# HuiHuiLan/Clustering-Hidden-Markov-Models-with-Variational-Bayesian-Hierarchical-EM

Hardware: AMD Instinct MI355X
Metric: VBHEM E-steps/sec (whole node), N baseHMMs × K clusters × S states; ELBO match (higher is better)
Workload: dtype f64; 1 GPU; C4: N=100000 base HMMs, K=16 clusters, S=8 states, Sb=8, d=8, full cov, tau=10, Nv=100; N=100000, K=16, S=8, Sb=8, d=8, tau=10, parallelism=bases sharded over 1 GPU(s), 1 RCCL all-reduce/E-step

## Files before the change

clustering-hidden-markov-models-with-variational-bayesian-hierarchical-em_amd/csrc/vbhem_capi.hip:

```cpp
#include <hip/hip_runtime.h>

#include <algorithm>
#include <atomic>
#include <chrono>
#include <cmath>
#include <cstdio>
#include <cstring>
#include <cstdlib>
#include <random>
#include <string>
#include <utility>
#include <vector>

#include "vbhem_estep.h"
#include "vbhem_internal.h"
#include "vbhem_exact.h"
#include "vbhem_math.h"

static std::atomic<size_t> g_debug_extra_lds{0};

namespace {

thread_local std::string g_err;

struct TimingState {
  int level = 0;
  std::vector<std::pair<hipEvent_t, hipEvent_t>> fb, stats, em, gf, emd;
  std::vector<long long> fb_pairs;
  std::vector<hipEvent_t> pool;
  ~TimingState() {
    for (hipEvent_t e : pool) (void)hipEventDestroy(e);
  }
};
thread_local TimingState g_timing;

thread_local std::string g_last_kernel[2];
std::string split_name(const vbhem::SplitArgs &a) {
  return "vbhem::fb_split_kernel<" + std::to_string(a.S) + ", " + std::to_string(a.lpc) + ", " +
         std::to_string(a.mode) + ">";
}

struct SwitchRow {
  const char *name;
  long long unset;
  long long vbhem::Switches::*field;
};
constexpr SwitchRow kSwitchRows[] = {
#define X(name, unset, doc) {"VBHEM_" #name, unset, &vbhem::Switches::name},
    VBHEM_SWITCHES(X)
#undef X
};
// ... 304 lines not shown
                     : nullptr;
  w.scratch = cv.take<double>(exact_stride(c->S, b->SB, T) * kExactThreads);
  return cv.off + 256;
}

struct FusedWs {
  int group;
  int nslab;
  int slab_len;
  int *fpre, *flags;
  int *gate_cnt, *list, *list_tot;
  double *Atg;
  double *scratch, *nu1, *xi, *tnu, *Z, *slabs;
  double *E, *W, *bias, *shift;
  double *U;
};

size_t carve_fused(void *ws, const vbhem_base_t *b, const vbhem_cluster_t *c, int T, FusedWs &w,
                   int R = 1) {
  Carver cv(ws);
  const int K = c->K, S = c->S, SB = b->SB;
  const size_t per_base = (size_t)K * (S + (size_t)S * S + 2 * (size_t)S * SB) * sizeof(double);
  size_t g = std::max<size_t>(1, kGroupBudget / std::max<size_t>(1, per_base));
  g = std::min<size_t>(g, (size_t)std::max(1, b->N));
  const vbhem::Switches &sw = vbhem::switches();
  if (sw.GROUP_BASES >= 0)
    g = std::max<size_t>(1, std::min<size_t>(g, (size_t)sw.GROUP_BASES));
  w.group = (int)g;
  int maxslab = kMaxSlabs;
  if (sw.NSLAB >= 0) maxslab = (int)std::max(1ll, std::min(8192ll, sw.NSLAB));
// ... 4 lines not shown
  w.nu1 = cv.take<double>(g * K * S);
  w.xi = cv.take<double>(g * K * S * S);
  w.tnu = cv.take<double>(g * K * S * SB);
  w.Z = cv.take<double>(g * K);
  w.slabs = cv.take<double>((size_t)w.nslab * w.slab_len);
  w.E = cv.take<double>(g * K * S * SB);
  w.W = cv.take<double>(emission_w_doubles(b->d, b->covmode, K, S));
  w.bias = cv.take<double>((size_t)vbhem::emission_ksp(K * S));
  w.shift = cv.take<double>((size_t)b->d);
  w.U = need_u_ws(b) ? cv.take<double>(vbhem::u_doubles((long long)g * SB + 16, b->d, b->covmode))
                     : nullptr;
  w.gate_cnt = cv.take<int>((size_t)w.nslab * K);
  w.list = cv.take<int>(g * K);
  w.list_tot = cv.take<int>((size_t)K);
  w.Atg = cv.take<double>((size_t)K * S * S);
  w.scratch = cv.take<double>(exact_stride(S, SB, T) * kExactThreads);
  return cv.off + 256;
}

struct FbCtx {
  FbPlan plan;
  SplitPlan split;
  SplitPlan bwd;
  size_t bwd2_lds = 0;
  int bwd2_ppb = 0, bwd2_nwb = 0;
  bool bwd12 = false;
  bool bwd4 = false;
  bool list4 = false;
  bool list12 = false;
  bool k1_in_kernel = false;
// ... 81 lines not shown
  c.em.Atg = Atg; c.em.logA = logA;
  hipError_t e = vbhem::launch_emission_prep(c.em, st);
  if (e != hipSuccess) return hip_fail(e, "emission_prep_kernel");
  return VBHEM_OK;
}

unsigned list_grid(const vbhem::SplitArgs &a, size_t lds) {
  const int cus = vbhem::device_cus();
  const int per_cu = std::max(1, vbhem::split_resident_blocks(a, lds));
  return (unsigned)(cus * per_cu);
}

int run_fb_list(const FbCtx &c, int i_begin, int i_end, int i_buf0, double *nu1, double *xi,
                double *tnu, const double *Ebuf, long long e_ld, const int *list,
                const int *list_tot, int list_cap, int *flags, double *scratch, double *LL,
                hipStream_t st, bool fold = false, bool *inlined = nullptr) {
  if (i_end <= i_begin) return VBHEM_OK;
  if (!c.split.lds_l) return fail(VBHEM_ERR_UNSUPPORTED, "gate-list pass does not fit LDS");
  vbhem::SplitArgs ca = c.split.al;
  ca.mode = vbhem::kFbList;
  ca.E = Ebuf; ca.e_ld = e_ld;
  ca.i_begin = i_begin; ca.i_end = i_end; ca.i_buf0 = i_buf0;
  ca.LL = nullptr; ca.nu1 = nu1; ca.xi = xi; ca.tnu = tnu;
  ca.flag_count = flags; ca.flag_list = flags + vbhem::kFlagHead;
  ca.list = list; ca.list_tot = list_tot; ca.list_cap = list_cap;
  ca.xinline = 0;
  auto set_inline = [&](long long waves) {
    if (!fold || waves > kExactThreads || vbhem::switches().NO_LIST_INLINE) return;
    ca.xinline = 1;
    ca.xscr = scratch;
    ca.xstride = (long long)exact_stride(c.plan.a.S, c.plan.a.SB, c.plan.a.T);
    vbhem::FbArgs &x = ca.xf;
    x = c.plan.a;
    x.i_begin = i_begin; x.i_end = i_end; x.i_buf0 = i_buf0;
    x.LL = LL; x.nu1 = nu1; x.xi = xi; x.tnu = tnu;
    x.flag_count = flags; x.flag_list = flags + vbhem::kFlagHead;
  };
  hipEvent_t ev0 = timing_on(st) ? timing_event(st) : nullptr;
  hipError_t e;
  if (c.list4) {
    ca.Atg = c.bwd.a.Atg;
    const unsigned grid = (unsigned)(vbhem::device_cus() * std::max(1, vbhem::list4_resident_blocks()));
    set_inline(vbhem::list4_inline_waves(ca, grid));
    e = vbhem::launch_list4(ca, grid, st);
    if (e != hipSuccess) return hip_fail(e, "fb_list4_kernel");
    g_last_kernel[1] = "vbhem::fb_list4_kernel<" + std::to_string(ca.T) +
                       (vbhem::list4_fast(ca) ? ", true>" : ", false>");
  } else if (c.list12) {
    ca.Atg = c.bwd.a.Atg;
    const unsigned grid = (unsigned)(vbhem::device_cus() * std::max(1, vbhem::list12_resident_blocks()));
    e = vbhem::launch_list12(ca, grid, st);
    if (e != hipSuccess) return hip_fail(e, "fb_list12_kernel");
    g_last_kernel[1] = "vbhem::fb_list12_kernel<" + std::to_string(ca.T) +
                       (vbhem::list12_fast(ca) ? ", true>" : ", false>");
  } else {
    if (c.k1_in_kernel) set_k1_operands(c, i_begin, ca);
    const unsigned grid = list_grid(ca, c.split.lds_l);
    if (ca.S >= vbhem::kSplitInlineMinS && ca.S <= vbhem::kSplitInlineMaxS)
// ... 139 lines not shown
  }
  e = vbhem::launch_fb_exact(a, scratch, exact_stride(a.S, a.SB, a.T), kExactThreads, st);
  if (e != hipSuccess) return hip_fail(e, "fb_exact_kernel");
  return VBHEM_OK;
}

}

extern "C" {

const char *vbhem_last_error(void) { return g_err.c_str(); }

size_t vbhem_debug_extra_lds(size_t bytes) { return g_debug_extra_lds.exchange(bytes); }

const char *vbhem_last_kernel(int pass) {
  return (pass == 0 || pass == 1) ? g_last_kernel[pass].c_str() : "";
}

const char *vbhem_version(void) { return "vbhem-mi355x 0.1.0 (gfx950)"; }

size_t vbhem_stats_nu(int d, int covmode) {
  return covmode == VBHEM_COV_FULL ? (size_t)1 + d + (size_t)d * (d + 1) / 2 : (size_t)1 + 2 * d;
}

size_t vbhem_stats_len(int K, int S, int d, int covmode) {
  return (size_t)K + (size_t)K * S + (size_t)K * S * S + 2 + (size_t)K * S * vbhem_stats_nu(d, covmode);
}

size_t vbhem_prepare_base_bytes(const vbhem_base_t *base) {
  if (!base || base->N < 0 || base->SB < 1 || base->d < 1 || base->d > vbhem::kUHead ||
      (base->covmode != VBHEM_COV_DIAG && base->covmode != VBHEM_COV_FULL))
// ... 284 lines not shown
        sa.U = base->U; sa.uz = base->U; sa.u_col0 = 0;
        sa.Us = base->U + vbhem::u_doubles((long long)base->N * SB, base->d, base->covmode);
      } else if (ctx.u_ws) {
        sa.U = ctx.u_ws; sa.uz = ctx.em.shift; sa.u_col0 = (long long)g0 * SB / 16 * 16;
      }
    }
    const int nchunk = std::max(1, chunks(g1 - g0));
    hipEvent_t ev0 = timing_on(st) ? timing_event(st) : nullptr;
    e = vbhem::launch_resp(sa, nchunk, st);
    if (e != hipSuccess) return hip_fail(e, "resp_kernel");
    if (gated) {
      e = vbhem::launch_gate_list(sa, nchunk, st);
      if (e != hipSuccess) return hip_fail(e, "gate_list_kernel");
      if (ev0) g_timing.stats.emplace_back(ev0, timing_event(st));
      bool inl = false;
      rc = run_fb_list(ctx, g0, g1, g0, w.nu1, w.xi, w.tnu, w.E, e_ld, w.list, w.list_tot,
                       w.group, w.flags, w.scratch, LL_elbo_dev, st, fold, &inl);
      if (rc != VBHEM_OK) return rc;
      if (fold) sa.fold = inl ? 2 : 1;
      ev0 = timing_on(st) ? timing_event(st) : nullptr;
      int ss = nchunk;
      e = vbhem::launch_stats_list(sa, nchunk, sl_lds, st, &ss);
      if (e != hipSuccess) return hip_fail(e, "stats_list_kernel");
      if (g0 == 0) stats_slabs = ss;
    } else {
      e = vbhem::launch_stats(sa, nchunk, ngroups, slds, st);
      if (e != hipSuccess) return hip_fail(e, "stats_kernel");
    }
    if (ev0) g_timing.stats.emplace_back(ev0, timing_event(st));
  }
  e = vbhem::launch_stats_final(w.slabs, nslab_used, stats_slabs, w.slab_len, sa.KT, S, sa.SL,
                                stats_dev, st, w.fpre, done_word, done_val);
  if (e != hipSuccess) return hip_fail(e, "stats_final_kernel");
  guard.fpre = nullptr;
  return VBHEM_OK;
}

// ... 426 lines not shown
```

clustering-hidden-markov-models-with-variational-bayesian-hierarchical-em_amd/csrc/vbhem_fb_list4.hip:

```cpp
#include <hip/hip_runtime.h>

#include <algorithm>
#include <cmath>
#include <type_traits>

#include "vbhem_exact.h"
#include "vbhem_internal.h"
#include "vbhem_math.h"
#include "vbhem_mfma4.h"


namespace vbhem {

namespace {
using namespace m4;
constexpr int kL4Waves = 2;
constexpr int kL4NWB = 4;
constexpr int kL4T = 10;
}
constexpr int kL4XQ = 1024;
namespace {
}

template <int T, bool FAST>
__global__ __launch_bounds__(64 * kL4NWB) __attribute__((amdgpu_waves_per_eu(kL4Waves)))
void fb_list4_kernel(const SplitArgs p) {
  constexpr int S = 8;
  __shared__ __attribute__((aligned(16))) double etab[2048];
  __shared__ __attribute__((aligned(16))) double ltab[2 * 1024];
  __shared__ int pre[kList4MaxK + 1];
  __shared__ int tots[kList4MaxK];
  __shared__ int xq[kL4NWB * kL4XQ];
  const int tid = threadIdx.x;
  stage_tables(etab, ltab, tid, 64 * kL4NWB);
  const int K = p.K, SB = FAST ? 8 : p.SB;
  using off_t_ = typename std::conditional<FAST, unsigned, size_t>::type;
  auto ld = [](const double *base, off_t_ x) {
    if constexpr (FAST)
      return *reinterpret_cast<const double *>(reinterpret_cast<const char *>(base) + x * 8u);
    else
      return base[x];
  };
  if (tid == 0) {
    int s = 0;
    for (int jj = 0; jj < K; ++jj) {
      const int t = p.list_tot[jj];
      pre[jj] = s;
      tots[jj] = t;
      s += (t + 3) / 4;
    }
    pre[K] = s;
  }
  __syncthreads();
  const int nitem = __builtin_amdgcn_readfirstlane(pre[K]);
  const double vlim = kVMax / (double)T - 3.0;
  const int gw = (int)blockIdx.x * kL4NWB + (tid >> 6), nw = (int)gridDim.x * kL4NWB;

  struct ItemIn {
    double ab[2][2], e[2][2], pr[2], af[2][2];
  };
  auto load_in = [&](int i, int jj, int r_, int c_, ItemIn &in) {
#pragma unroll
    for (int j2 = 0; j2 < 2; ++j2)
#pragma unroll
      for (int j3 = 0; j3 < 2; ++j3) {
        const int be = 4 * j3 + c_, bp = 4 * j2 + r_;
        const int bec = be < SB ? be : SB - 1, bpc = bp < SB ? bp : SB - 1;
        in.ab[j2][j3] = ld(p.A, ((off_t_)i * SB + bec) * SB + bpc);
        in.af[j2][j3] = ld(p.A, ((off_t_)i * SB + bpc) * SB + bec);
      }
#pragma unroll
// ... 6 lines not shown
      }
#pragma unroll
    for (int j3 = 0; j3 < 2; ++j3) {
      const int be = 4 * j3 + c_;
      in.pr[j3] = ld(p.prior, (off_t_)i * SB + (be < SB ? be : SB - 1));
    }
  };
  auto base_of = [&](int it, int jj, int b_) -> int {
    const int n0 = (it - pre[jj]) * 4;
    const int tot = tots[jj];
    return p.list[(size_t)jj * p.list_cap + (n0 + b_ < tot ? n0 + b_ : n0)];
  };
  int js = 0, jsn = 0, nq = 0;
  ItemIn cur;
  int icur = 0;
  if (gw < nitem) {
    const int lane = tid & 63;
    while (pre[js + 1] <= gw) ++js;
    jsn = js;
    icur = base_of(gw, __builtin_amdgcn_readfirstlane(js), (lane >> 2) & 3);
    load_in(icur, __builtin_amdgcn_readfirstlane(js), lane >> 4, lane & 3, cur);
  }
  for (int it = gw; it < nitem; it += nw) {
    int tq = tid;
    asm volatile("" : "+v"(tq));
    const int lane = tq & 63;
    const int r = lane >> 4, b = (lane >> 2) & 3, c = lane & 3;
    const int qsrc0 = (4 * b + r) << 2, qsrc1 = (16 + 4 * b + r) << 2;
    const int taddr = (16 * c + 4 * b + r) << 2;
    const unsigned long long pmask = 0x000F000F000F000Full << (4 * b);
    const int j = __builtin_amdgcn_readfirstlane(js);
    const int itn = min(it + nw, nitem - 1);
    while (pre[jsn + 1] <= itn) ++jsn;
    const int jn = __builtin_amdgcn_readfirstlane(jsn);
    const int inext = base_of(itn, jn, b);
    double AT[2][2], Ap[2][2], amQ[2], lpP[2];
    bool cl_nf;
    {
      const double *At = p.Atg + (size_t)j * S * S;
      bool nf = false;
#pragma unroll
      for (int x = 0; x < 2; ++x)
#pragma unroll
        for (int y = 0; y < 2; ++y) {
          AT[x][y] = At[(4 * y + c) * S + 4 * x + r];
          Ap[x][y] = At[(4 * x + r) * S + 4 * y + c];
        }
// ... 125 lines not shown
        wpf[x] = 2147483648u - kBias;
      }
      exp_m_n<4>(ef, xf, sf, wpf, etab);
#pragma unroll
      for (int jj = 0; jj < 2; ++jj) {
        const int be = 4 * jj + c;
        const double pb = be < SB ? cur.pr[jj] : 0.0;
        nu[0][jj] = pb * ef[jj];
        nu[1][jj] = pb * ef[2 + jj];
      }
#pragma unroll
      for (int i2 = 0; i2 < 2; ++i2) {
        double a = nu[i2][0] + nu[i2][1];
        a += shfl_xor_d(a, 1);
        a += shfl_xor_d(a, 2);
        if (act && c == 0) p.nu1[lp * S + 4 * i2 + r] = a;
      }
    }

    double AbF[2][2];
#pragma unroll
    for (int j2 = 0; j2 < 2; ++j2)
#pragma unroll
      for (int jj = 0; jj < 2; ++jj) {
        const int bp = 4 * j2 + r, be = 4 * jj + c;
        AbF[j2][jj] = (be < SB && bp < SB) ? cur.af[j2][jj] : 0.0;
      }
    ItemIn nxt;
    double nuT[2][2], tnT[2][2], H[2][2];
    transpose8(nu, nuT, taddr);
#pragma unroll
    for (int x = 0; x < 2; ++x)
#pragma unroll
      for (int y = 0; y < 2; ++y) {
        tnT[x][y] = nuT[x][y];
        H[x][y] = 0.0;
      }
#pragma unroll
    for (int t = 1; t < T; ++t) {
      if (t == T / 2) load_in(inext, jn, r, c, nxt);
      double Gt[2][2];
      transpose8(lat[t], Gt, taddr);
      double fT[2][2], ZT[2][2];
#pragma unroll
      for (int jj = 0; jj < 2; ++jj)
#pragma unroll
        for (int i2 = 0; i2 < 2; ++i2) {
          fT[jj][i2] = mfma4(AbF[1][jj], nuT[1][i2], mfma4(AbF[0][jj], nuT[0][i2], 0.0));
          ZT[jj][i2] = mfma4(lat[t][1][jj], AT[1][i2], mfma4(lat[t][0][jj], AT[0][i2], 0.0));
        }
      double gT[2][2];
      {
        const double zf[4] = {ZT[0][0], ZT[0][1], ZT[1][0], ZT[1][1]};
        double rz[4];
        rcp_pos_n<4>(rz, zf);
// ... 6 lines not shown
        for (int i3 = 0; i3 < 2; ++i3) H[i2][i3] = mfma4(gT[1][i2], Gt[1][i3], mfma4(gT[0][i2], Gt[0][i3], H[i2][i3]));
      double g[2][2];
      transpose8(gT, g, taddr);
#pragma unroll
      for (int jj = 0; jj < 2; ++jj)
#pragma unroll
        for (int i3 = 0; i3 < 2; ++i3) {
          const double qm = mfma4(g[1][jj], Ap[1][i3], mfma4(g[0][jj], Ap[0][i3], 0.0));
          nuT[jj][i3] = Gt[jj][i3] * qm;
          tnT[jj][i3] += nuT[jj][i3];
        }
    }

    const bool pbad = (__ballot(bad) & pmask) != 0;
    const bool pnf = cl_nf || (__ballot(nfp) & pmask) != 0;
    if (act) {
#pragma unroll
      for (int jj = 0; jj < 2; ++jj)
#pragma unroll
        for (int i2 = 0; i2 < 2; ++i2) {
          const int be = 4 * jj + r;
          if (be < SB) p.tnu[(lp * S + 4 * i2 + c) * SB + be] = tnT[jj][i2];
        }
#pragma unroll
      for (int i2 = 0; i2 < 2; ++i2)
#pragma unroll
        for (int i3 = 0; i3 < 2; ++i3) p.xi[(lp * S + 4 * i2 + r) * S + 4 * i3 + c] = Ap[i2][i3] * H[i2][i3];
      if (pbad && !pnf && lane == 4 * b) {
        atomicAdd(p.flag_count + 1, 1);
        if (!p.xinline) {
          const int slot = atomicAdd(p.flag_count, 1);
          p.flag_list[slot] = (int)((size_t)i * K + j);
        }
      }
    }
    if (p.xinline) {
      const unsigned long long fm = __ballot(act && pbad && !pnf && lane == 4 * b);
      if (fm) {
        const int l = (int)__builtin_amdgcn_mbcnt_hi((unsigned)(fm >> 32), __builtin_amdgcn_mbcnt_lo((unsigned)fm, 0u));
        if (fm >> lane & 1) xq[(tid >> 6) * kL4XQ + nq + l] = (int)((size_t)i * K + j);
        nq += __builtin_popcountll(fm);
      }
    }
    cur = nxt;
    icur = inext;
    js = jsn;
  }
  if (p.xinline) {
    const int *q = xq + (tid >> 6) * kL4XQ;
    for (int x = 0; x < nq; ++x)
      exact_pair_wave<true>(p.xf, __builtin_amdgcn_readfirstlane(q[x]), p.xscr + (size_t)gw * p.xstride, nullptr);
  }
}

bool list4_supported(int S, int SB, int T, int K) {
  return S == 8 && SB >= 1 && SB <= 8 && T == kL4T && K >= 1 && K <= kList4MaxK;
}
bool list4_fast(const SplitArgs &a) {
  const unsigned long long lim = 0xffffffffull / 8;
  return a.SB == 8 && (unsigned long long)a.i_end * a.SB * a.SB < lim &&
         (unsigned long long)a.K * a.S * (unsigned long long)a.e_ld < lim;
}
long long list4_inline_waves(const SplitArgs &a, unsigned grid) {
  const long long nw = (long long)grid * kL4NWB;
  const long long items = (long long)a.K * ((a.i_end - a.i_begin + 3) / 4);
  if (nw < 1 || 4 * ((items + nw - 1) / nw) > kL4XQ) return 1ll << 40;
  return nw;
}
int list4_resident_blocks() {
  auto *fn = &fb_list4_kernel<kL4T, true>;
  return resident_per_cu(reinterpret_cast<const void *>(fn), 64 * kL4NWB, 0);
}
hipError_t launch_list4(const SplitArgs &a, unsigned grid, hipStream_t st) {
  if (!list4_supported(a.S, a.SB, a.T, a.K) || !a.Atg || !a.list || !a.list_tot) return hipErrorInvalidValue;
  auto *fn = list4_fast(a) ? &fb_list4_kernel<kL4T, true> : &fb_list4_kernel<kL4T, false>;
  hipLaunchKernelGGL(fn, dim3(grid), dim3(64 * kL4NWB), 0, st, a);
  return hipGetLastError();
}

}
```

clustering-hidden-markov-models-with-variational-bayesian-hierarchical-em_amd/csrc/vbhem_internal.h:

```cpp
#pragma once
#include <hip/hip_runtime.h>

#include <cstddef>
#include <map>
#include <mutex>
#include <string>
#include <tuple>

#include "vbhem_estep.h"
#include "vbhem_switches.h"

namespace vbhem {

int set_error(int code, const std::string &msg);
static inline int hip_fail(hipError_t e, const char *where) {
  return set_error(VBHEM_ERR_HIP, std::string(where) + ": " + hipGetErrorString(e));
}

static inline size_t align_up(size_t x, size_t a) { return (x + a - 1) / a * a; }

inline int current_device() {
  int dev = 0;
  if (hipGetDevice(&dev) != hipSuccess) dev = 0;
  return dev;
}
// ... 196 lines not shown
  int list_cap;
  const double *Atg;
  const double *eU, *eW, *ebias;
  long long e_col0;
  int ekdp, eksp;
  double esmooth;
  int xinline;
  double *xscr;
  long long xstride;
  FbArgs xf;
  int prep;
  const double *pm, *pP, *pc, *pz;
  double *pshift;
  unsigned long long *ftag;
  unsigned long long ftag_val;
};

constexpr double kLog2PiE = 1.8378770664093454835606594728112353;
__device__ __forceinline__ double em_psym(const double *P, int a, int b, int d) {
  return 0.5 * (P[a * d + b] + P[b * d + a]);
}
__device__ __forceinline__ double em_pm_full(const double *P, const double *mr, const double *zs,
                                             int a, int d) {
  double v = 0.0;
  for (int b = 0; b < d; ++b) v = fma(em_psym(P, a, b, d), mr[b] - zs[b], v);
  return v;
}
__device__ __forceinline__ double em_w_full(const double *P, int a, int b, int d) {
  return -0.5 * ((a == b) ? P[a * d + a] : em_psym(P, a, b, d));
}
// ... 43 lines not shown
int bwd4_resident_blocks();
bool bwd4_o32(const SplitArgs &a);
bool bwd12_o32(const SplitArgs &a);
bool list4_fast(const SplitArgs &a);
bool list12_fast(const SplitArgs &a);
hipError_t launch_bwd4(const SplitArgs &a, unsigned grid, hipStream_t st, hipEvent_t t0 = nullptr,
                       hipEvent_t t1 = nullptr);
bool bwd12_supported(int S, int SB);
int bwd12_ppb();
int bwd12_resident_blocks();
hipError_t launch_bwd12(const SplitArgs &a, unsigned grid, hipStream_t st, hipEvent_t t0 = nullptr,
                        hipEvent_t t1 = nullptr);

constexpr int kList4MaxK = 1024;
bool list4_supported(int S, int SB, int T, int K);
int list4_resident_blocks();
long long list4_inline_waves(const SplitArgs &a, unsigned grid);
hipError_t launch_list4(const SplitArgs &a, unsigned grid, hipStream_t st);

bool list12_supported(int S, int SB, int T, int K);
int list12_resident_blocks();
hipError_t launch_list12(const SplitArgs &a, unsigned grid, hipStream_t st);

hipError_t launch_fb(const FbArgs &a, dim3 grid, dim3 block, size_t lds, hipStream_t st);
constexpr int kFlagHead = 4;
constexpr int kFlagPre = 4;
constexpr int kFlagLost = 3;
constexpr int kFlagLostMark = 0x4C4F5354;
unsigned long long flag_tag();
constexpr int kFlagBad = 1, kFlagNonFinite = 2;
#ifndef VBHEM_EXACT_BLOCK
#define VBHEM_EXACT_BLOCK 512
#endif
// ... 22 lines not shown
```

clustering-hidden-markov-models-with-variational-bayesian-hierarchical-em_amd/csrc/vbhem_stats.hip:

```cpp
#include <hip/hip_runtime.h>

#include <algorithm>
#include <cmath>
#include <cstdlib>

#include "vbhem_internal.h"
#include "vbhem_exact.h"

namespace vbhem {

namespace {

typedef double double4_t __attribute__((ext_vector_type(4)));

__device__ __forceinline__ double wave_max(double v) {
#pragma unroll
  for (int off = 32; off >= 1; off >>= 1) v = fmax(v, __shfl_xor(v, off, 64));
  return v;
}
__device__ __forceinline__ double wave_sum(double v) {
#pragma unroll
  for (int off = 32; off >= 1; off >>= 1) v += __shfl_xor(v, off, 64);
  return v;
}
// ... 1000 lines not shown
  const int ntiles = ((RG + 15) / 16) * ((a.NU + 15) / 16);
  const int tpw = (ntiles + kStatsWaves - 1) / kStatsWaves;
  if (a.vhem) {
    if (tpw <= 4) return launch_stats_t<4, kGateVhem>(a, nchunk, ngroups, lds, st);
    if (tpw <= 8) return launch_stats_t<8, kGateVhem>(a, nchunk, ngroups, lds, st);
    return launch_stats_t<16, kGateVhem>(a, nchunk, ngroups, lds, st);
  }
  if (tpw <= 4) return launch_stats_t<4, kGateVbhem>(a, nchunk, ngroups, lds, st);
  if (tpw <= 8) return launch_stats_t<8, kGateVbhem>(a, nchunk, ngroups, lds, st);
  return launch_stats_t<16, kGateVbhem>(a, nchunk, ngroups, lds, st);
}

constexpr int kSuWaves = 4;

__device__ __forceinline__ void su_output(const StatsArgs &p, const double *red, const double *zs,
                                          int c, int nch, int j, int tid) {
  const int S = p.S, NU = p.NU, d = p.d;
  const bool full = p.covmode == kCovFull;
  const int KT = p.KT, tr = j / KT, jt = j - tr * KT;
  double *tsl = p.slabs + (size_t)c * p.slab_len + (size_t)tr * p.SL;
  const int NO = S * NU + S + S * S;
  for (int o = tid; o < NO; o += 64 * kSuWaves) {
    double v;
    double *dst;
    if (o < S * NU) {
      const int s2 = o / NU, f = o - s2 * NU;
      const double *rs = red + (size_t)s2 * NU;
      const double N = rs[0];
      if (f == 0) {
        v = N;
      } else if (f <= d) {
        v = fma(zs[f - 1], N, rs[f]);
      } else {
        int a = f - 1 - d, b = a;
        if (full) {
          int k = a;
          a = 0;
          while (k >= d - a) { k -= d - a; ++a; }
          b = a + k;
// ... 296 lines not shown
      }
#pragma unroll
      for (int r = 0; r < NXR; ++r) {
        const int x = lane + 64 * (tg + TG * r);
        if (x < NX) {
          double *o = red + (size_t)S * NU + x;
          *o = g == 0 ? ax[r] : *o + ax[r];
        }
      }
    }
    __syncthreads();
  }
  su_output(p, red, zs, c, nch, j, tid);
}

template <int LG, int SM>
__global__ __launch_bounds__(64 * kSuWaves) void stats_list_g_kernel(const StatsArgs p) {
  extern __shared__ double lds[];
  constexpr int NG = 64 / LG;
  const int tid = threadIdx.x, lane = tid & 63, wave = tid >> 6;
  const int grp = lane / LG, gl = lane - grp * LG;
  const int K = p.K, S = p.S, SB = p.SB, d = p.d, NU = p.NU, kq = p.ukdp / 4;
  const bool full = p.covmode == kCovFull;
  const int NPF = full ? d * (d + 1) / 2 : d;
  const int j = blockIdx.y, c = blockIdx.x, nch = gridDim.x;
  const int OT = S * SB, TS = (OT + 1) / 2 * 2, KP = p.ukdp + 1;
  const int WS = TS + (SB * KP + 1) / 2 * 2;
  double *tw = lds + (size_t)(wave * NG + grp) * WS;
  double *uw = tw + TS;
  double *red = lds + (size_t)kSuWaves * NG * WS;
// ... 272 lines not shown
    }
    if (a.NU <= 64) return launch_su_s<1>(b, g2, st);
    if (a.NU <= 128) return launch_su_s<2>(b, g2, st);
    return launch_su_s<3>(b, g2, st);
  }
  if (NO <= 4 * kSlThreads) {
    hipLaunchKernelGGL((stats_list_kernel<4>), grid, dim3(kSlThreads), lds, st, a);
  } else {
    hipError_t e = set_dyn_lds(reinterpret_cast<const void *>(&stats_list_kernel<8>), lds);
    if (e != hipSuccess) return e;
    hipLaunchKernelGGL((stats_list_kernel<8>), grid, dim3(kSlThreads), lds, st, a);
  }
  return hipGetLastError();
}

hipError_t launch_stats_final(const double *slabs, int nslab, int nslab_stats, int slab_len, int KT,
                              int S, int SL, double *out, hipStream_t st, int *fpre,
                              unsigned long long *done, unsigned long long done_val) {
  if (nslab_stats < 1 || nslab_stats > nslab || SL < 1 || slab_len % SL != 0) return hipErrorInvalidValue;
  hipLaunchKernelGGL(stats_final_kernel, dim3((slab_len + kFinalCols - 1) / kFinalCols), dim3(256),
                     0, st, slabs, nslab, nslab_stats, slab_len, KT, S, SL, out, fpre,
                     fpre ? flag_tag() : 0ull, fpre ? done : nullptr, done_val);
  return hipGetLastError();
}

}
```

clustering-hidden-markov-models-with-variational-bayesian-hierarchical-em_amd/csrc/vbhem_switches.h:

```cpp
#pragma once

#define VBHEM_SWITCHES(X)                                                                      \
  X(FUSED_DENSE, 0, "dense schedule instead of the gated one (vbhem_set_fused_mode)")          \
  X(NO_UGEMM, 0, "emission on the raw / generic kernels instead of the prepared operand")      \
  X(GROUP_BASES, -1, "tests: at most n bases per group of the fused call")                     \
  X(NSLAB, -1, "tests: at most n statistics slabs (1 .. 8192)")                                \
  X(NO_BWD2, 0, "backward pass on fb_split_kernel's backward mode, not fb_bwd2_kernel")        \
  X(NO_BWD4, 0, "S = 8: fb_bwd2_kernel<8> instead of fb_bwd4_kernel")                          \
  X(NO_BWD12, 0, "S = 12: fb_bwd2_kernel<12> instead of fb_bwd12_kernel")                      \
  X(NO_LIST4, 0, "S = 8: fb_split_kernel's list mode instead of fb_list4_kernel")              \
  X(NO_LIST12, 0, "S = 12: fb_split_kernel's list mode instead of fb_list12_kernel")           \
  X(NO_K1_IN_KERNEL, 0, "short K1 through the emission GEMM, not inside the recursion")        \
  X(NO_LIST_INLINE, 0, "the gate-list pass's flagged pairs through an fb_exact_kernel launch") \
  X(NO_BWD2_PREP, 0, "emission_prep_kernel launched, not its work inside fb_bwd2_kernel")      \
  X(NO_FOLD_EXACT, 0, "the backward pass's fallback as a launch, not folded into resp_kernel") \
  X(EM_NOBST, 0, "the one-chunk emission GEMM without buffer stores")                          \
  X(EM_SPLIT, -1, "the one-chunk emission GEMM in whole (0) or half (1) tiles")                \
  X(EM_NODB, 0, "the chunked emission GEMM on emission_u_kernel, not emission_db_kernel")      \
  X(RESP_GENERIC, 0, "resp_kernel's generic path for every K")                                 \
  X(SU_BLOCKS, -1, "gated statistics: the block count")                                        \
  X(NO_STATS_G, 0, "gated statistics: no lane-grouped kernel")                                 \
  X(NO_STATS_U, 0, "gated statistics: the covariance-gather kernel")                           \
  X(NO_STATS_M, 0, "gated statistics: without stats_list_m_kernel")                            \
  X(STATS_U, 0, "gated statistics: the prepared-operand kernel at any NU")                     \
  X(EM_HOST_MATH, 0, "the EM loop's per-iteration math on the host")

namespace vbhem {
// ... 11 lines not shown
```

Baseline: 555.1 E-steps/s.

## Accumulate sufficient statistics inside fb_list4_kernel and reduce per-wave partials

For S=8 with the list4 gate-list pass, the forward-backward kernel now accumulates the weighted statistics (nu1, xi, tnu times U) in LDS per wave, using MFMA, instead of writing per-pair outputs. Each wave is assigned a contiguous range of items and flushes partial sums into slots, which a new reduce kernel sums and emits through su_output. This replaces the separate stats_list kernel and the global round-trip of per-pair nu1, xi and tnu. In exchange it adds LDS usage, register pressure, possibly lower residency, and a second reduction pass over the slots.

```diff
diff --git a/clustering-hidden-markov-models-with-variational-bayesian-hierarchical-em_amd/csrc/vbhem_capi.hip b/clustering-hidden-markov-models-with-variational-bayesian-hierarchical-em_amd/csrc/vbhem_capi.hip
--- a/clustering-hidden-markov-models-with-variational-bayesian-hierarchical-em_amd/csrc/vbhem_capi.hip
+++ b/clustering-hidden-markov-models-with-variational-bayesian-hierarchical-em_amd/csrc/vbhem_capi.hip
@@ -34,7 +34,7 @@
 };
 thread_local TimingState g_timing;
 
-thread_local std::string g_last_kernel[2];
+thread_local std::string g_last_kernel[3];
 std::string split_name(const vbhem::SplitArgs &a) {
   return "vbhem::fb_split_kernel<" + std::to_string(a.S) + ", " + std::to_string(a.lpc) + ", " +
          std::to_string(a.mode) + ">";
@@ -369,6 +369,7 @@
   double *scratch, *nu1, *xi, *tnu, *Z, *slabs;
   double *E, *W, *bias, *shift;
   double *U;
+  double *l4parts;
 };
 
 size_t carve_fused(void *ws, const vbhem_base_t *b, const vbhem_cluster_t *c, int T, FusedWs &w,
@@ -403,6 +404,11 @@
   w.list = cv.take<int>(g * K);
   w.list_tot = cv.take<int>((size_t)K);
   w.Atg = cv.take<double>((size_t)K * S * S);
+  const int NU = (int)vbhem_stats_nu(b->d, b->covmode);
+  w.l4parts = vbhem::list4_acc_supported(S, SB, T, K, NU)
+                  ? cv.take<double>((size_t)vbhem::l4s_max_slots(kExactThreads, K) *
+                                    vbhem::l4s_part_len(S, vbhem::us_nup(NU)))
+                  : nullptr;
   w.scratch = cv.take<double>(exact_stride(S, SB, T) * kExactThreads);
   return cv.off + 256;
 }
@@ -514,7 +520,9 @@
 int run_fb_list(const FbCtx &c, int i_begin, int i_end, int i_buf0, double *nu1, double *xi,
                 double *tnu, const double *Ebuf, long long e_ld, const int *list,
                 const int *list_tot, int list_cap, int *flags, double *scratch, double *LL,
-                hipStream_t st, bool fold = false, bool *inlined = nullptr) {
+                hipStream_t st, bool fold = false, bool *inlined = nullptr,
+                const vbhem::StatsArgs *acc_sa = nullptr, double *acc_parts = nullptr,
+                int *acc_waves = nullptr) {
   if (i_end <= i_begin) return VBHEM_OK;
   if (!c.split.lds_l) return fail(VBHEM_ERR_UNSUPPORTED, "gate-list pass does not fit LDS");
   vbhem::SplitArgs ca = c.split.al;
@@ -525,8 +533,13 @@
   ca.flag_count = flags; ca.flag_list = flags + vbhem::kFlagHead;
   ca.list = list; ca.list_tot = list_tot; ca.list_cap = list_cap;
   ca.xinline = 0;
+  const vbhem::Switches &sw = vbhem::switches();
+  const bool acc = c.list4 && acc_sa && acc_parts && acc_sa->Us && acc_sa->Z && !acc_sa->vhem &&
+                   vbhem::list4_acc_supported(ca.S, ca.SB, ca.T, ca.K, acc_sa->NU) &&
+                   !sw.NO_LIST4_STATS && !sw.NO_STATS_M && !sw.NO_STATS_U;
+  if (acc_waves) *acc_waves = 0;
   auto set_inline = [&](long long waves) {
-    if (!fold || waves > kExactThreads || vbhem::switches().NO_LIST_INLINE) return;
+    if (!(fold || (acc && !sw.NO_FOLD_EXACT)) || waves > kExactThreads || sw.NO_LIST_INLINE) return;
     ca.xinline = 1;
     ca.xscr = scratch;
     ca.xstride = (long long)exact_stride(c.plan.a.S, c.plan.a.SB, c.plan.a.T);
@@ -540,8 +553,17 @@
   hipError_t e;
   if (c.list4) {
     ca.Atg = c.bwd.a.Atg;
-    const unsigned grid = (unsigned)(vbhem::device_cus() * std::max(1, vbhem::list4_resident_blocks()));
+    unsigned grid = (unsigned)(vbhem::device_cus() * std::max(1, vbhem::list4_resident_blocks(acc)));
     set_inline(vbhem::list4_inline_waves(ca, grid));
+    if (acc && ca.xinline) {
+      ca.acc = 1;
+      ca.acc_nup = vbhem::us_nup(acc_sa->NU);
+      ca.accZ = acc_sa->Z; ca.accUs = acc_sa->Us; ca.acc_parts = acc_parts;
+      if (acc_waves) *acc_waves = (int)vbhem::list4_inline_waves(ca, grid);
+    } else if (acc) {
+      grid = (unsigned)(vbhem::device_cus() * std::max(1, vbhem::list4_resident_blocks()));
+      if (fold) set_inline(vbhem::list4_inline_waves(ca, grid));
+    }
     e = vbhem::launch_list4(ca, grid, st);
     if (e != hipSuccess) return hip_fail(e, "fb_list4_kernel");
     g_last_kernel[1] = "vbhem::fb_list4_kernel<" + std::to_string(ca.T) +
@@ -711,7 +733,7 @@
 size_t vbhem_debug_extra_lds(size_t bytes) { return g_debug_extra_lds.exchange(bytes); }
 
 const char *vbhem_last_kernel(int pass) {
-  return (pass == 0 || pass == 1) ? g_last_kernel[pass].c_str() : "";
+  return (pass >= 0 && pass <= 2) ? g_last_kernel[pass].c_str() : "";
 }
 
 const char *vbhem_version(void) { return "vbhem-mi355x 0.1.0 (gfx950)"; }
@@ -1026,13 +1048,22 @@
       if (e != hipSuccess) return hip_fail(e, "gate_list_kernel");
       if (ev0) g_timing.stats.emplace_back(ev0, timing_event(st));
       bool inl = false;
+      int l4w = 0;
       rc = run_fb_list(ctx, g0, g1, g0, w.nu1, w.xi, w.tnu, w.E, e_ld, w.list, w.list_tot,
-                       w.group, w.flags, w.scratch, LL_elbo_dev, st, fold, &inl);
+                       w.group, w.flags, w.scratch, LL_elbo_dev, st, fold, &inl, &sa, w.l4parts, &l4w);
       if (rc != VBHEM_OK) return rc;
       if (fold) sa.fold = inl ? 2 : 1;
       ev0 = timing_on(st) ? timing_event(st) : nullptr;
       int ss = nchunk;
-      e = vbhem::launch_stats_list(sa, nchunk, sl_lds, st, &ss);
+      if (l4w > 0) {
+        ss = 1;
+        g_last_kernel[2] = "vbhem::list4_stats_reduce_kernel";
+        e = vbhem::launch_list4_stats_reduce(sa, w.l4parts, l4w, st);
+        if (e != hipSuccess) return hip_fail(e, "list4_stats_reduce_kernel");
+      } else {
+        g_last_kernel[2] = "vbhem::stats_list_kernels";
+        e = vbhem::launch_stats_list(sa, nchunk, sl_lds, st, &ss);
+      }
       if (e != hipSuccess) return hip_fail(e, "stats_list_kernel");
       if (g0 == 0) stats_slabs = ss;
     } else {
diff --git a/clustering-hidden-markov-models-with-variational-bayesian-hierarchical-em_amd/csrc/vbhem_fb_list4.hip b/clustering-hidden-markov-models-with-variational-bayesian-hierarchical-em_amd/csrc/vbhem_fb_list4.hip
--- a/clustering-hidden-markov-models-with-variational-bayesian-hierarchical-em_amd/csrc/vbhem_fb_list4.hip
+++ b/clustering-hidden-markov-models-with-variational-bayesian-hierarchical-em_amd/csrc/vbhem_fb_list4.hip
@@ -20,9 +20,94 @@
 }
 constexpr int kL4XQ = 1024;
 namespace {
-}
-
-template <int T, bool FAST>
+constexpr int kL4AccM = 2 * kL4sMaxTiles * 64, kL4AccN = kL4AccM + 4 * 64, kL4AccS = kL4AccN + 32;
+constexpr int kL4AccLen = kL4AccS + 32;
+#ifndef VBHEM_L4_US_T0
+#define VBHEM_L4_US_T0 8
+#endif
+#ifndef VBHEM_L4_US_T1
+#define VBHEM_L4_US_T1 10
+#endif
+
+__device__ __forceinline__ void l4_wsync() {
+  __builtin_amdgcn_fence(__ATOMIC_RELEASE, "wavefront");
+  __builtin_amdgcn_wave_barrier();
+  __builtin_amdgcn_fence(__ATOMIC_ACQUIRE, "wavefront");
+}
+__device__ __forceinline__ void l4_load_us(const SplitArgs &p, int i, int sbp, int ntile, int lane,
+                                           double (&ub)[kL4sMaxTiles][2]) {
+  const double *us = p.accUs + (size_t)i * sbp * p.acc_nup + lane;
+#pragma unroll
+  for (int f = 0; f < kL4sMaxTiles; ++f)
+#pragma unroll
+    for (int J = 0; J < 2; ++J) ub[f][J] = us[((f < ntile ? f : ntile - 1) * sbp + (4 * J < sbp ? 4 * J : 0)) * 16];
+}
+template <int NP>
+__device__ __forceinline__ void l4_acc_u(double *accw, const double (&za)[2][2],
+                                         const double (&ub)[NP][kL4sMaxTiles][2], int r, int c, int lane) {
+  double acc[2][kL4sMaxTiles];
+#pragma unroll
+  for (int I = 0; I < 2; ++I)
+#pragma unroll
+    for (int f = 0; f < kL4sMaxTiles; ++f) acc[I][f] = accw[(I * kL4sMaxTiles + f) * 64 + lane];
+#pragma unroll
+  for (int pp = 0; pp < NP; ++pp) {
+    const int src = (16 * r + 4 * pp + c) << 2;
+#pragma unroll
+    for (int J = 0; J < 2; ++J)
+#pragma unroll
+      for (int I = 0; I < 2; ++I) {
+        const double xa = bperm_d(src, za[J][I]);
+#pragma unroll
+        for (int f = 0; f < kL4sMaxTiles; ++f) acc[I][f] = mfma4(xa, ub[pp][f][J], acc[I][f]);
+      }
+  }
+#pragma unroll
+  for (int I = 0; I < 2; ++I)
+#pragma unroll
+    for (int f = 0; f < kL4sMaxTiles; ++f) accw[(I * kL4sMaxTiles + f) * 64 + lane] = acc[I][f];
+}
+__device__ __forceinline__ void l4_acc_nm(double *accw, const double (&n1)[2], const double (&xm)[2][2],
+                                          int r, int b, int c, int lane) {
+#pragma unroll
+  for (int I = 0; I < 2; ++I) {
+    if (c == 0) accw[kL4AccN + 16 * I + 4 * r + b] += n1[I];
+#pragma unroll
+    for (int I2 = 0; I2 < 2; ++I2) accw[kL4AccM + (2 * I + I2) * 64 + lane] += xm[I][I2];
+  }
+}
+__device__ __forceinline__ void l4_flush(const SplitArgs &p, double *accw, int slot, bool add, int ntile,
+                                         int lane) {
+  constexpr int S = 8;
+  const int nup = p.acc_nup, r = lane >> 4, b = (lane >> 2) & 3, c = lane & 3;
+  double *part = p.acc_parts + (size_t)slot * l4s_part_len(S, nup);
+  auto put = [add](double *dst, double v) { *dst = add ? *dst + v : v; };
+#pragma unroll
+  for (int I = 0; I < 2; ++I)
+#pragma unroll
+    for (int f = 0; f < kL4sMaxTiles; ++f) {
+      double *a = accw + (I * kL4sMaxTiles + f) * 64 + lane;
+      if (f < ntile) put(part + (4 * I + r) * nup + 16 * f + 4 * b + c, *a);
+      *a = 0.0;
+    }
+  l4_wsync();
+  {
+    const double *a = accw + kL4AccM + (2 * (lane >> 5) + ((lane >> 2) & 1)) * 64 + 16 * ((lane >> 3) & 3) + (lane & 3);
+    put(part + S * nup + S + lane, ((a[0] + a[4]) + a[8]) + a[12]);
+  }
+  if (lane < S) {
+    const double *a = accw + kL4AccN + 16 * (lane >> 2) + 4 * (lane & 3);
+    put(part + S * nup + lane, ((a[0] + a[1]) + a[2]) + a[3]);
+  }
+  l4_wsync();
+#pragma unroll
+  for (int x = 0; x < 4; ++x) accw[kL4AccM + 64 * x + lane] = 0.0;
+  if (lane < 32) accw[kL4AccN + lane] = 0.0;
+  l4_wsync();
+}
+}
+
+template <int T, bool FAST, bool ACC>
 __global__ __launch_bounds__(64 * kL4NWB) __attribute__((amdgpu_waves_per_eu(kL4Waves)))
 void fb_list4_kernel(const SplitArgs p) {
   constexpr int S = 8;
@@ -31,8 +116,11 @@
   __shared__ int pre[kList4MaxK + 1];
   __shared__ int tots[kList4MaxK];
   __shared__ int xq[kL4NWB * kL4XQ];
+  __shared__ __attribute__((aligned(16))) double accs[ACC ? kL4NWB * kL4AccLen : 1];
   const int tid = threadIdx.x;
   stage_tables(etab, ltab, tid, 64 * kL4NWB);
+  if constexpr (ACC)
+    for (int x = tid; x < kL4NWB * kL4AccLen; x += 64 * kL4NWB) accs[x] = 0.0;
   const int K = p.K, SB = FAST ? 8 : p.SB;
   using off_t_ = typename std::conditional<FAST, unsigned, size_t>::type;
   auto ld = [](const double *base, off_t_ x) {
@@ -54,7 +142,9 @@
   __syncthreads();
   const int nitem = __builtin_amdgcn_readfirstlane(pre[K]);
   const double vlim = kVMax / (double)T - 3.0;
-  const int gw = (int)blockIdx.x * kL4NWB + (tid >> 6), nw = (int)gridDim.x * kL4NWB;
+  const int gw = ACC ? __builtin_amdgcn_readfirstlane((int)blockIdx.x * kL4NWB + (tid >> 6))
+                     : (int)blockIdx.x * kL4NWB + (tid >> 6),
+            nw = (int)gridDim.x * kL4NWB;
 
   struct ItemIn {
     double ab[2][2], e[2][2], pr[2], af[2][2];
@@ -91,23 +181,27 @@
   int js = 0, jsn = 0, nq = 0;
   ItemIn cur;
   int icur = 0;
-  if (gw < nitem) {
+  const int per = ACC ? l4s_per_wave(nitem, nw) : 1;
+  const int it0 = ACC ? gw * per : gw, itend = ACC ? min(nitem, it0 + per) : nitem;
+  const int istep = ACC ? 1 : nw;
+  if (it0 < itend) {
     const int lane = tid & 63;
-    while (pre[js + 1] <= gw) ++js;
+    while (pre[js + 1] <= it0) ++js;
     jsn = js;
-    icur = base_of(gw, __builtin_amdgcn_readfirstlane(js), (lane >> 2) & 3);
+    icur = base_of(it0, __builtin_amdgcn_readfirstlane(js), (lane >> 2) & 3);
     load_in(icur, __builtin_amdgcn_readfirstlane(js), lane >> 4, lane & 3, cur);
   }
-  for (int it = gw; it < nitem; it += nw) {
+  for (int it = it0; it < itend; it += istep) {
     int tq = tid;
     asm volatile("" : "+v"(tq));
     const int lane = tq & 63;
     const int r = lane >> 4, b = (lane >> 2) & 3, c = lane & 3;
+    double *const accw = accs + (ACC ? (tq >> 6) * kL4AccLen : 0);
     const int qsrc0 = (4 * b + r) << 2, qsrc1 = (16 + 4 * b + r) << 2;
     const int taddr = (16 * c + 4 * b + r) << 2;
     const unsigned long long pmask = 0x000F000F000F000Full << (4 * b);
     const int j = __builtin_amdgcn_readfirstlane(js);
-    const int itn = min(it + nw, nitem - 1);
+    const int itn = min(it + istep, itend - 1);
     while (pre[jsn + 1] <= itn) ++jsn;
     const int jn = __builtin_amdgcn_readfirstlane(jsn);
     const int inext = base_of(itn, jn, b);
@@ -263,7 +357,11 @@
         double a = nu[i2][0] + nu[i2][1];
         a += shfl_xor_d(a, 1);
         a += shfl_xor_d(a, 2);
-        if (act && c == 0) p.nu1[lp * S + 4 * i2 + r] = a;
+        if constexpr (ACC) {
+          if (c == 0) accw[kL4AccS + 16 * i2 + 4 * r + b] = a;
+        } else {
+          if (act && c == 0) p.nu1[lp * S + 4 * i2 + r] = a;
+        }
       }
     }
 
@@ -276,6 +374,9 @@
         AbF[j2][jj] = (be < SB && bp < SB) ? cur.af[j2][jj] : 0.0;
       }
     ItemIn nxt;
+    double zc = 0.0, ub[ACC ? 4 : 1][kL4sMaxTiles][2];
+    const int sbp = us_sbp(SB), ntile = ACC ? p.acc_nup / 16 : 1;
+    if constexpr (ACC) zc = p.accZ[lp];
     double nuT[2][2], tnT[2][2], H[2][2];
     transpose8(nu, nuT, taddr);
 #pragma unroll
@@ -288,6 +389,16 @@
 #pragma unroll
     for (int t = 1; t < T; ++t) {
       if (t == T / 2) load_in(inext, jn, r, c, nxt);
+      if constexpr (ACC)
+        if (t == VBHEM_L4_US_T0) {
+          l4_load_us(p, __builtin_amdgcn_readlane(i, 0), sbp, ntile, lane, ub[0]);
+          l4_load_us(p, __builtin_amdgcn_readlane(i, 4), sbp, ntile, lane, ub[1]);
+        }
+      if constexpr (ACC)
+        if (t == VBHEM_L4_US_T1) {
+          l4_load_us(p, __builtin_amdgcn_readlane(i, 8), sbp, ntile, lane, ub[2]);
+          l4_load_us(p, __builtin_amdgcn_readlane(i, 12), sbp, ntile, lane, ub[3]);
+        }
       double Gt[2][2];
       transpose8(lat[t], Gt, taddr);
       double fT[2][2], ZT[2][2];
@@ -324,7 +435,27 @@
 
     const bool pbad = (__ballot(bad) & pmask) != 0;
     const bool pnf = cl_nf || (__ballot(nfp) & pmask) != 0;
-    if (act) {
+    if constexpr (ACC) {
+      if (VBHEM_L4_US_T1 >= T) {
+        l4_load_us(p, __builtin_amdgcn_readlane(i, 8), sbp, ntile, lane, ub[2]);
+        l4_load_us(p, __builtin_amdgcn_readlane(i, 12), sbp, ntile, lane, ub[3]);
+      }
+      const bool use = act && !(pbad && !pnf);
+      double za[2][2], xm[2][2], n1[2];
+#pragma unroll
+      for (int x = 0; x < 2; ++x) {
+        n1[x] = use ? zc * accw[kL4AccS + 16 * x + 4 * r + b] : 0.0;
+#pragma unroll
+        for (int y = 0; y < 2; ++y) {
+          za[x][y] = (use && (FAST || 4 * x + r < SB)) ? zc * tnT[x][y] : 0.0;
+          xm[x][y] = use ? zc * (Ap[x][y] * H[x][y]) : 0.0;
+        }
+      }
+      l4_acc_nm(accw, n1, xm, r, b, c, lane);
+      l4_acc_u<4>(accw, za, ub, r, c, lane);
+      if (act && pbad && !pnf && lane == 4 * b) atomicAdd(p.flag_count + 1, 1);
+      if (it + 1 >= itend || jn != j) l4_flush(p, accw, l4s_slot(it, j, per), false, ntile, lane);
+    } else if (act) {
 #pragma unroll
       for (int jj = 0; jj < 2; ++jj)
 #pragma unroll
@@ -348,7 +479,7 @@
       const unsigned long long fm = __ballot(act && pbad && !pnf && lane == 4 * b);
       if (fm) {
         const int l = (int)__builtin_amdgcn_mbcnt_hi((unsigned)(fm >> 32), __builtin_amdgcn_mbcnt_lo((unsigned)fm, 0u));
-        if (fm >> lane & 1) xq[(tid >> 6) * kL4XQ + nq + l] = (int)((size_t)i * K + j);
+        if (fm >> lane & 1) xq[((ACC ? tq : tid) >> 6) * kL4XQ + nq + l] = (int)((size_t)i * K + j);
         nq += __builtin_popcountll(fm);
       }
     }
@@ -358,8 +489,39 @@
   }
   if (p.xinline) {
     const int *q = xq + (tid >> 6) * kL4XQ;
-    for (int x = 0; x < nq; ++x)
-      exact_pair_wave<true>(p.xf, __builtin_amdgcn_readfirstlane(q[x]), p.xscr + (size_t)gw * p.xstride, nullptr);
+    for (int x = 0; x < nq; ++x) {
+      const int pair = __builtin_amdgcn_readfirstlane(q[x]);
+      exact_pair_wave<true>(p.xf, pair, p.xscr + (size_t)gw * p.xstride, nullptr);
+      if constexpr (ACC) {
+        __builtin_amdgcn_fence(__ATOMIC_SEQ_CST, "agent");
+        __builtin_amdgcn_wave_barrier();
+        int tq = tid;
+        asm volatile("" : "+v"(tq));
+        const int lane = tq & 63, r = lane >> 4, b = (lane >> 2) & 3, c = lane & 3;
+        double *const accw = accs + (tq >> 6) * kL4AccLen;
+        const int i = pair / K, j = pair - i * K;
+        const size_t lp = (size_t)(i - p.i_buf0) * K + j;
+        const int sbp = us_sbp(SB), ntile = p.acc_nup / 16;
+        const bool on = b == 0;
+        const double zc = p.accZ[lp];
+        double ub[1][kL4sMaxTiles][2], za[2][2], xm[2][2], n1[2];
+        l4_load_us(p, i, sbp, ntile, lane, ub[0]);
+#pragma unroll
+        for (int x2 = 0; x2 < 2; ++x2) {
+          n1[x2] = on ? zc * p.nu1[lp * S + 4 * x2 + r] : 0.0;
+#pragma unroll
+          for (int y = 0; y < 2; ++y) {
+            const bool tv = on && 4 * x2 + r < SB;
+            za[x2][y] = tv ? zc * p.tnu[(lp * S + 4 * y + c) * SB + 4 * x2 + r] : 0.0;
+            xm[x2][y] = on ? zc * p.xi[(lp * S + 4 * x2 + r) * S + 4 * y + c] : 0.0;
+          }
+        }
+        l4_acc_nm(accw, n1, xm, r, b, c, lane);
+        l4_acc_u<1>(accw, za, ub, r, c, lane);
+        const int jx = x + 1 < nq ? __builtin_amdgcn_readfirstlane(q[x + 1]) % K : -1;
+        if (jx != j) l4_flush(p, accw, gw + j, true, ntile, lane);
+      }
+    }
   }
 }
 
@@ -377,15 +539,40 @@
   if (nw < 1 || 4 * ((items + nw - 1) / nw) > kL4XQ) return 1ll << 40;
   return nw;
 }
-int list4_resident_blocks() {
-  auto *fn = &fb_list4_kernel<kL4T, true>;
+bool list4_acc_supported(int S, int SB, int T, int K, int NU) {
+  return list4_supported(S, SB, T, K) && us_nup(NU) <= 16 * kL4sMaxTiles;
+}
+int list4_resident_blocks(bool acc) {
+  auto *fn = acc ? &fb_list4_kernel<kL4T, true, true> : &fb_list4_kernel<kL4T, true, false>;
   return resident_per_cu(reinterpret_cast<const void *>(fn), 64 * kL4NWB, 0);
 }
 hipError_t launch_list4(const SplitArgs &a, unsigned grid, hipStream_t st) {
   if (!list4_supported(a.S, a.SB, a.T, a.K) || !a.Atg || !a.list || !a.list_tot) return hipErrorInvalidValue;
-  auto *fn = list4_fast(a) ? &fb_list4_kernel<kL4T, true> : &fb_list4_kernel<kL4T, false>;
+  auto *fn = list4_fast(a) ? &fb_list4_kernel<kL4T, true, false> : &fb_list4_kernel<kL4T, false, false>;
+  if (a.acc) {
+    if (!a.xinline || !a.accZ || !a.accUs || !a.acc_parts || a.acc_nup < 16 || a.acc_nup % 16 ||
+        a.acc_nup > 16 * kL4sMaxTiles)
+      return hipErrorInvalidValue;
+    fn = list4_fast(a) ? &fb_list4_kernel<kL4T, true, true> : &fb_list4_kernel<kL4T, false, true>;
+  }
   hipLaunchKernelGGL(fn, dim3(grid), dim3(64 * kL4NWB), 0, st, a);
   return hipGetLastError();
 }
 
 }
+
+extern "C" int vbhem_list4_stats_slot_plan(const int *tot, int K, int nw, int *per, int *first,
+                                           int *count) {
+  int nitem = 0;
+  for (int j = 0; j < K; ++j) nitem += vbhem::l4s_items(tot[j]);
+  const int pw = vbhem::l4s_per_wave(nitem, nw);
+  if (per) *per = pw;
+  int pre = 0;
+  for (int j = 0; j < K; ++j) {
+    const int n = vbhem::l4s_items(tot[j]);
+    if (first) first[j] = n ? vbhem::l4s_slot(pre, j, pw) : 0;
+    if (count) count[j] = n ? vbhem::l4s_slot(pre + n - 1, j, pw) - vbhem::l4s_slot(pre, j, pw) + 1 : 0;
+    pre += n;
+  }
+  return nitem;
+}
diff --git a/clustering-hidden-markov-models-with-variational-bayesian-hierarchical-em_amd/csrc/vbhem_internal.h b/clustering-hidden-markov-models-with-variational-bayesian-hierarchical-em_amd/csrc/vbhem_internal.h
--- a/clustering-hidden-markov-models-with-variational-bayesian-hierarchical-em_amd/csrc/vbhem_internal.h
+++ b/clustering-hidden-markov-models-with-variational-bayesian-hierarchical-em_amd/csrc/vbhem_internal.h
@@ -9,6 +9,7 @@
 
 #include "vbhem_estep.h"
 #include "vbhem_switches.h"
+#include "vbhem_list4_slots.h"
 
 namespace vbhem {
 
@@ -235,6 +236,11 @@
   double *pshift;
   unsigned long long *ftag;
   unsigned long long ftag_val;
+  int acc;
+  int acc_nup;
+  const double *accZ;
+  const double *accUs;
+  double *acc_parts;
 };
 
 constexpr double kLog2PiE = 1.8378770664093454835606594728112353;
@@ -308,9 +314,11 @@
 
 constexpr int kList4MaxK = 1024;
 bool list4_supported(int S, int SB, int T, int K);
-int list4_resident_blocks();
+int list4_resident_blocks(bool acc = false);
 long long list4_inline_waves(const SplitArgs &a, unsigned grid);
 hipError_t launch_list4(const SplitArgs &a, unsigned grid, hipStream_t st);
+bool list4_acc_supported(int S, int SB, int T, int K, int NU);
+hipError_t launch_list4_stats_reduce(const StatsArgs &a, const double *parts, int nw, hipStream_t st);
 
 bool list12_supported(int S, int SB, int T, int K);
 int list12_resident_blocks();
diff --git a/clustering-hidden-markov-models-with-variational-bayesian-hierarchical-em_amd/csrc/vbhem_list4_slots.h b/clustering-hidden-markov-models-with-variational-bayesian-hierarchical-em_amd/csrc/vbhem_list4_slots.h
--- /dev/null
+++ b/clustering-hidden-markov-models-with-variational-bayesian-hierarchical-em_amd/csrc/vbhem_list4_slots.h
@@ -0,0 +1,20 @@
+#pragma once
+#include <hip/hip_runtime.h>
+
+namespace vbhem {
+
+constexpr int kL4sMaxTiles = 3;
+
+__host__ __device__ inline int l4s_items(int tot) { return (tot + 3) / 4; }
+__host__ __device__ inline int l4s_per_wave(int nitem, int nw) {
+  return nitem > 0 && nw > 0 ? (nitem + nw - 1) / nw : 1;
+}
+__host__ __device__ inline int l4s_wave(int item, int per) { return item / per; }
+__host__ __device__ inline int l4s_slot(int item, int cluster, int per) { return item / per + cluster; }
+__host__ __device__ inline int l4s_max_slots(int nw, int K) { return nw + K; }
+__host__ __device__ inline int l4s_part_len(int S, int NUP) { return S * NUP + S + S * S; }
+
+}
+
+extern "C" int vbhem_list4_stats_slot_plan(const int *tot, int K, int nw, int *per, int *first,
+                                           int *count);
diff --git a/clustering-hidden-markov-models-with-variational-bayesian-hierarchical-em_amd/csrc/vbhem_stats.hip b/clustering-hidden-markov-models-with-variational-bayesian-hierarchical-em_amd/csrc/vbhem_stats.hip
--- a/clustering-hidden-markov-models-with-variational-bayesian-hierarchical-em_amd/csrc/vbhem_stats.hip
+++ b/clustering-hidden-markov-models-with-variational-bayesian-hierarchical-em_amd/csrc/vbhem_stats.hip
@@ -1038,7 +1038,7 @@
 constexpr int kSuWaves = 4;
 
 __device__ __forceinline__ void su_output(const StatsArgs &p, const double *red, const double *zs,
-                                          int c, int nch, int j, int tid) {
+                                          int c, int nch, int j, int tid, int row = -1) {
   const int S = p.S, NU = p.NU, d = p.d;
   const bool full = p.covmode == kCovFull;
   const int KT = p.KT, tr = j / KT, jt = j - tr * KT;
@@ -1047,6 +1047,7 @@
   for (int o = tid; o < NO; o += 64 * kSuWaves) {
     double v;
     double *dst;
+    if (row >= 0 && (o < S * NU ? o / NU : o < S * NU + S ? o - S * NU : (o - S * NU - S) / S) != row) continue;
     if (o < S * NU) {
       const int s2 = o / NU, f = o - s2 * NU;
       const double *rs = red + (size_t)s2 * NU;
@@ -1373,6 +1374,60 @@
   su_output(p, red, zs, c, nch, j, tid);
 }
 
+constexpr int kL4rParts = 16, kL4rCols = 64, kL4rThreads = kL4rParts * kL4rCols;
+__global__ __launch_bounds__(kL4rThreads) void list4_stats_reduce_kernel(const StatsArgs p,
+                                                                        const double *parts, int nw) {
+  extern __shared__ double lds[];
+  __shared__ int plan[2];
+  __shared__ double part[kL4rParts][kL4rCols];
+  const int tid = threadIdx.x, S = p.S, j = blockIdx.x / S, s2 = blockIdx.x - j * S;
+  const int NU = p.NU, NUP = us_nup(NU), d = p.d;
+  if (tid == 0) {
+    int nitem = 0, pre = 0;
+    for (int x = 0; x < p.K; ++x) {
+      if (x == j) pre = nitem;
+      nitem += l4s_items(p.list_tot[x]);
+    }
+    const int per = l4s_per_wave(nitem, nw), n = l4s_items(p.list_tot[j]);
+    plan[0] = l4s_slot(pre, j, per);
+    plan[1] = n ? l4s_slot(pre + n - 1, j, per) - plan[0] + 1 : 0;
+  }
+  __syncthreads();
+  const int s0 = plan[0], ns = plan[1];
+  const int NO = S * NU + S + S * S, PL = l4s_part_len(S, NUP);
+  double *red = lds;
+  double *zs = red + NO;
+  for (int a = tid; a < d; a += kL4rThreads) zs[a] = p.uz[a];
+  const int q = tid / kL4rCols, col = tid - q * kL4rCols;
+  const bool cv = col < NU + 1 + S;
+  const int src = col < NU ? s2 * NUP + col : col == NU ? S * NUP + s2 : S * NUP + S + s2 * S + (col - NU - 1);
+  const int dst = col < NU ? s2 * NU + col : col == NU ? S * NU + s2 : S * NU + S + s2 * S + (col - NU - 1);
+  const int k0 = (int)((long long)ns * q / kL4rParts), k1 = (int)((long long)ns * (q + 1) / kL4rParts);
+  double acc = 0.0;
+  if (cv) {
+    const double *g = parts + (size_t)s0 * PL + src;
+    int k = k0;
+    for (; k + 7 < k1; k += 8) {
+      double v[8];
+#pragma unroll
+      for (int u = 0; u < 8; ++u) v[u] = g[(size_t)(k + u) * PL];
+#pragma unroll
+      for (int u = 0; u < 8; ++u) acc += v[u];
+    }
+    for (; k < k1; ++k) acc += g[(size_t)k * PL];
+  }
+  part[q][col] = acc;
+  __syncthreads();
+  if (q == 0 && cv) {
+    double t = part[0][col];
+#pragma unroll
+    for (int x = 1; x < kL4rParts; ++x) t += part[x][col];
+    red[dst] = t;
+  }
+  __syncthreads();
+  if (tid < 64 * kSuWaves) su_output(p, red, zs, 0, 1, j, tid, s2);
+}
+
 template <int LG, int SM>
 __global__ __launch_bounds__(64 * kSuWaves) void stats_list_g_kernel(const StatsArgs p) {
   extern __shared__ double lds[];
@@ -1675,6 +1730,16 @@
   return hipGetLastError();
 }
 
+hipError_t launch_list4_stats_reduce(const StatsArgs &a, const double *parts, int nw, hipStream_t st) {
+  if (!parts || nw < 1 || !a.uz || !a.list_tot) return hipErrorInvalidValue;
+  StatsArgs b = a;
+  b.nzero = 1;
+  if (a.NU + 1 + a.S > kL4rCols) return hipErrorInvalidValue;
+  const size_t lds = ((size_t)(a.S * a.NU + a.S + a.S * a.S) + a.d) * sizeof(double);
+  hipLaunchKernelGGL(list4_stats_reduce_kernel, dim3(a.K * a.S), dim3(kL4rThreads), lds, st, b, parts, nw);
+  return hipGetLastError();
+}
+
 hipError_t launch_stats_final(const double *slabs, int nslab, int nslab_stats, int slab_len, int KT,
                               int S, int SL, double *out, hipStream_t st, int *fpre,
                               unsigned long long *done, unsigned long long done_val) {
diff --git a/clustering-hidden-markov-models-with-variational-bayesian-hierarchical-em_amd/csrc/vbhem_switches.h b/clustering-hidden-markov-models-with-variational-bayesian-hierarchical-em_amd/csrc/vbhem_switches.h
--- a/clustering-hidden-markov-models-with-variational-bayesian-hierarchical-em_amd/csrc/vbhem_switches.h
+++ b/clustering-hidden-markov-models-with-variational-bayesian-hierarchical-em_amd/csrc/vbhem_switches.h
@@ -11,6 +11,7 @@
   X(NO_LIST4, 0, "S = 8: fb_split_kernel's list mode instead of fb_list4_kernel")              \
   X(NO_LIST12, 0, "S = 12: fb_split_kernel's list mode instead of fb_list12_kernel")           \
   X(NO_K1_IN_KERNEL, 0, "short K1 through the emission GEMM, not inside the recursion")        \
+  X(NO_LIST4_STATS, 0, "S = 8: per-pair outputs + stats_list_m_kernel, not sums in fb_list4_kernel") \
   X(NO_LIST_INLINE, 0, "the gate-list pass's flagged pairs through an fb_exact_kernel launch") \
   X(NO_BWD2_PREP, 0, "emission_prep_kernel launched, not its work inside fb_bwd2_kernel")      \
   X(NO_FOLD_EXACT, 0, "the backward pass's fallback as a launch, not folded into resp_kernel") \
```

Result: faster. 581.0 E-steps/s (median of 6 runs) (+4.7%).
